# Geronimorz/MCMC-in-Tonga

Measured on AMD Instinct MI355X. Metric: MCMC proposals/sec (likelihood evals/sec) at 381 rays x N cells, higher is better.
Workload: dtype f64

## Files before the change

include/tdstar_testing.h:

```cpp
#ifndef TDSTAR_TESTING_H
#define TDSTAR_TESTING_H
#include <stdint.h>

#include "tdstar.h"

#ifdef __cplusplus
extern "C" {
#endif

void tdt_philox(const uint32_t ctr[4], const uint32_t key[2], uint32_t out[4]);
double tdt_det_log(double x);
double tdt_det_exp(double x);
double tdt_normal_quantile(double p);
void tdt_draws(uint64_t seed, uint32_t chain, uint64_t iter, double out[7]);
int tdt_propose(const td_chain_params *prm, uint64_t iter, int64_t ncells, const double *cx, const double *cy,
                const double *cz, const double *czeta, double czeta_birth, double out[8]);
int tdt_chain_profile(td_chain *ch, int enable, int64_t out[80]);
int tdt_chain_lds(td_chain *ch, int64_t out[4]);
int tdt_chain_variant(const int64_t in[15], int64_t out[8]);
int tdt_chain_variant_rounds(const int64_t in[15], int rounds_rec, int64_t out[8]);
int tdt_chain_launch_counts(int64_t out[32], int *n);
int tdt_chain_draws_launches(int64_t *n);
int tdt_history_pack(int device, double *cells, int64_t stride, int64_t slot0, int64_t slot_cells,
                     const int32_t *ncells, int64_t count, int64_t *off_out);
int tdt_history_pack_chunk(void);
int tdt_chain_query_lat(td_chain *ch, const double *pts, int nq, int mode, int64_t out[4]);
int tdt_tile_filter(const float *lo, const float *hi, const double *maxd, int nt, const double *queries, int nq,
                    int mode, uint8_t *hit);
int tdt_chain_query_answers(td_chain *ch, const double *pts, int nq, int mode, double *dist, double *value,
                            int32_t *proven);
int tdt_accept(const td_chain_params *prm, int action, double u_accept, double zeta_new, int64_t ncells, double phi,
               double phi_n, double czeta, double zeta_killed, double zetanew_death);
int tdt_decide_sure(const td_chain_params *prm, int action, double u_accept, double zeta_new, int64_t ncells,
// ... 64 lines not shown
```

mcmc-in-tonga_amd/_lib.py:

```python
import ctypes
import os

import numpy as np

HERE = os.path.dirname(os.path.abspath(__file__))
LIB_PATH = os.environ.get("TD_LIB_PATH") or os.path.join(HERE, "libtdstar.so")

TD_OK, TD_ERR_ARG, TD_ERR_LAYOUT, TD_ERR_HIP, TD_ERR_NOMEM, TD_ERR_BOUNDS = range(6)
TD_ENGINE_DEVICE, TD_ENGINE_HOST, TD_ENGINE_DROPIN = 0, 1, 2

_d = ctypes.c_double
_i32 = ctypes.c_int32
_i64 = ctypes.c_int64
_u32 = ctypes.c_uint32
_u64 = ctypes.c_uint64
_pd = ctypes.POINTER(ctypes.c_double)
_pi32 = ctypes.POINTER(ctypes.c_int32)
_pi64 = ctypes.POINTER(ctypes.c_int64)
_pu32 = ctypes.POINTER(ctypes.c_uint32)
_vp = ctypes.c_void_p


class TdInfo(ctypes.Structure):
    _fields_ = [("abi_version", _i32), ("device", _i32), ("m", _i64), ("n", _i64), ("npoints", _i64),
# ... 118 lines not shown
    "tdt_set_volume_counting": (ctypes.c_int, [_vp, ctypes.c_int]),
    "tdt_convergence_plan": (ctypes.c_int, [_i64, _pi64, _i64, _pi64, _pi64, _pd]),
    "tdt_set_convergence_round": (ctypes.c_int, [_vp, _i64]),
    "tdt_set_convergence_lag_block": (ctypes.c_int, [_vp, ctypes.c_int]),
    "tdt_quantile_rank": (ctypes.c_int, [_i64, _d, _pi64, _pd]),
    "tdt_set_marginals_method": (ctypes.c_int, [_vp, ctypes.c_int]),
    "tdt_marginals_resident_max": (ctypes.c_int, [_vp, _pi64]),
    "tdt_philox": (None, [_pu32, _pu32, _pu32]),
    "tdt_det_log": (_d, [_d]),
    "tdt_det_exp": (_d, [_d]),
    "tdt_normal_quantile": (_d, [_d]),
    "tdt_draws": (None, [_u64, _u32, _u64, _pd]),
    "tdt_propose": (ctypes.c_int, [ctypes.POINTER(TdChainParams), _u64, _i64, _pd, _pd, _pd, _pd, _d, _pd]),
    "tdt_chain_profile": (ctypes.c_int, [_vp, ctypes.c_int, _pi64]),
    "tdt_chain_lds": (ctypes.c_int, [_vp, _pi64]),
    "tdt_chain_variant": (ctypes.c_int, [_pi64, _pi64]),
    "tdt_chain_variant_rounds": (ctypes.c_int, [_pi64, ctypes.c_int, _pi64]),
    "tdt_chain_launch_counts": (ctypes.c_int, [_pi64, ctypes.POINTER(ctypes.c_int)]),
    "tdt_chain_draws_launches": (ctypes.c_int, [_pi64]),
    "tdt_history_pack": (ctypes.c_int, [ctypes.c_int, _pd, _i64, _i64, _i64, _pi32, _i64, _pi64]),
    "tdt_history_pack_chunk": (ctypes.c_int, []),
    "tdt_chain_query_lat": (ctypes.c_int, [_vp, _pd, ctypes.c_int, ctypes.c_int, _pi64]),
    "tdt_chain_query_answers": (ctypes.c_int, [_vp, _pd, ctypes.c_int, ctypes.c_int, _pd, _pd, _pi32]),
    "tdt_tile_filter": (ctypes.c_int, [ctypes.POINTER(ctypes.c_float), ctypes.POINTER(ctypes.c_float), _pd,
                                       ctypes.c_int, _pd, ctypes.c_int, ctypes.c_int,
                                       ctypes.POINTER(ctypes.c_uint8)]),
    "tdt_set_nn_method": (ctypes.c_int, [_vp, ctypes.c_int]),
    "tdt_nn_bench": (ctypes.c_int, [_vp, _pd, _pd, _pd, _pd, _i64, ctypes.c_int, ctypes.c_int, _pd]),
    "tdt_chain_set_lds_mode": (ctypes.c_int, [_vp, ctypes.c_int]),
    "tdt_chain_set_exact_every": (ctypes.c_int, [_vp, ctypes.c_int]),
# ... 69 lines not shown
```

mcmc-in-tonga_amd/csrc/chain.cpp:

```cpp
#include <hip/hip_runtime.h>

#include <algorithm>
#include <atomic>
#include <chrono>
#include <climits>
#include <cmath>
#include <cstdlib>
#include <cstdio>
#include <cstring>
#include <new>
#include <string>
#include <mutex>
#include <thread>
#include <vector>

#include "../../include/tdstar_testing.h"
#include "chain_dev.h"
#include "chain_logic.h"
#include "comm.h"
#include "ctx.h"
#include "history.h"

using namespace tdstar;

// ... 331 lines not shown
        const int b = grid_bucket(G, ch->x[i], ch->y[i], ch->z[i]);
        if (bcount[(size_t)b] < kBucketCap) {
            bslot[(size_t)b * kBucketCap + bcount[(size_t)b]] = (int)i;
            bent[(size_t)b * kBucketCap + bcount[(size_t)b]++] = CellEntry{ch->x[i], ch->y[i], ch->z[i], ch->zeta[i]};
        }
        else
            overflow = 1;
    }
    size_t bytes = 0;
    auto add = [&](size_t b) { bytes += ((b + 255) / 256) * 256; };
    const size_t Pn = (size_t)std::max<int64_t>(P, 1), nn = (size_t)std::max<int64_t>(n, 1);
    add(sizeof(int) * (ntiles + 1)); add(sizeof(int) * (ntiles + 1)); add(sizeof(int) * Pn);
    add(sizeof(float) * 3 * ntiles); add(sizeof(float) * 3 * ntiles); add(sizeof(double) * (ntiles + 1)); add(sizeof(double) * (ntiles + 1));
    add(sizeof(float) * 3 * std::max(nsuper, 1)); add(sizeof(float) * 3 * std::max(nsuper, 1));
    add(sizeof(double) * 4 * cap); add(sizeof(double) * (cap + 2)); for (int i = 0; i < 3; ++i) add(sizeof(int) * cap); add(sizeof(long long) * cap);
    add(sizeof(int) * Pn); add(sizeof(double) * Pn); add(sizeof(double) * Pn);
    add(sizeof(int) * Pn); add(sizeof(double) * Pn); add(sizeof(double) * Pn); add(Pn);
    add(sizeof(int) * Pn); add(sizeof(int) * Pn); add(sizeof(int) * (ntiles + 1));
    for (int i = 0; i < 6; ++i) add(sizeof(double) * nn);
    add(sizeof(int) * nn); add(sizeof(int) * nn); add(sizeof(ChainScalars));
    add(sizeof(int) * nbuckets); add(sizeof(CellEntry) * nbuckets * kBucketCap); add(sizeof(int) * nbuckets * kBucketCap); add(sizeof(int));
    add(sizeof(DevChain));
    hipError_t e = hipMalloc(&ch->dev_block, bytes);
    if (e != hipSuccess) return hip_err(c, e, "hipMalloc(chain state)");
    e = hipMemsetAsync(ch->dev_block, 0, bytes, c->stream);
    if (e != hipSuccess) return hip_err(c, e, "hipMemset(chain state)");
    char *cur = (char *)ch->dev_block;
    DevChain &d = ch->dev;
    d.px = c->g.px; d.py = c->g.py; d.pz = c->g.pz; d.w = c->g.w; d.tS = c->g.tS; d.sig = c->g.sig;
    d.ray_off = c->g.ray_off;
    d.P = (int)P;
// ... 6 lines not shown
    d.tile_start = tile_start; d.tile_ray = tile_ray_d; d.pt_ray = pt_ray_d; d.tile_lo = tlo; d.tile_hi = thi;
    d.tile_maxd = carve<double>(cur, ntiles + 1);
    d.tile_cmax = carve<double>(cur, ntiles + 1);
    d.ntiles = ntiles;
    float *slo_d = carve<float>(cur, 3 * (size_t)std::max(nsuper, 1));
    float *shi_d = carve<float>(cur, 3 * (size_t)std::max(nsuper, 1));
    d.super_lo = slo_d; d.super_hi = shi_d; d.nsuper = nsuper;
    double *cells = carve<double>(cur, 4 * (size_t)cap);
    d.cx = cells; d.cy = cells + cap; d.cz = cells + 2 * cap; d.czeta = cells + 3 * cap;
    double *logN_d = carve<double>(cur, (size_t)cap + 2);
    d.logN = logN_d;
    d.order = carve<int>(cur, cap); d.stamp = carve<long long>(cur, cap);
    d.free_slots = carve<int>(cur, cap); d.order_tmp = carve<int>(cur, cap);
    d.cap = cap;
    d.best_s = carve<int>(cur, Pn); d.best_d = carve<double>(cur, Pn); d.zeta0 = carve<double>(cur, Pn);
    d.cand_s = carve<int>(cur, Pn); d.cand_d = carve<double>(cur, Pn); d.cand_z = carve<double>(cur, Pn);
    d.cand_flag = carve<unsigned char>(cur, Pn);
    d.changed = carve<int>(cur, Pn); d.orphans = carve<int>(cur, Pn); d.tiles_hit = carve<int>(cur, ntiles + 1);
    d.ptS = carve<double>(cur, nn); d.cand_ptS = carve<double>(cur, nn);
    d.prefix = carve<double>(cur, nn); d.cand_prefix = carve<double>(cur, nn);
    d.term = carve<double>(cur, nn); d.cand_term = carve<double>(cur, nn);
    d.rays_hit = carve<int>(cur, nn); d.ray_flag = carve<int>(cur, nn);
    d.st = carve<ChainScalars>(cur, 1);
    d.grid = G;
    d.bucket_count = carve<int>(cur, nbuckets);
    d.buckets = carve<CellEntry>(cur, nbuckets * kBucketCap);
    d.bslot = carve<int>(cur, nbuckets * kBucketCap);
    d.grid_overflow = carve<int>(cur, 1);
    ch->dev_ptr = carve<DevChain>(cur, 1);
    ch->st_dev = d.st;
// ... 1531 lines not shown
}
int tdt_chain_set_lds_mode(td_chain *ch, int mode) {
    if (!ch || ch->engine != TD_ENGINE_DEVICE || mode < 0 || mode > 3) return TD_ERR_ARG;
    ch->dev.lds_mode = mode;
    ch->desc_dirty = true;
    return TD_OK;
}

int tdt_chain_set_exact_every(td_chain *ch, int k) {
    if (!ch || ch->engine != TD_ENGINE_DEVICE || k < 0) return TD_ERR_ARG;
    ch->dev.exact_every = k;
    ch->desc_dirty = true;
    return TD_OK;
}

int tdt_chain_lds(td_chain *ch, int64_t out[4]) {
    if (!ch || ch->engine != TD_ENGINE_DEVICE || !out) return TD_ERR_ARG;
    chain_lds_sizes(ch->dev, out);
    return TD_OK;
}

int tdt_chain_query_lat(td_chain *ch, const double *pts, int nq, int mode, int64_t out[4]) {
    if (!ch || ch->engine != TD_ENGINE_DEVICE || !pts || nq < 1 || !out) return TD_ERR_ARG;
    td_ctx *c = ch->ctx;
    double *dp = nullptr;
    long long *dout = nullptr;
    hipError_t e = hipMalloc((void **)&dp, sizeof(double) * 3 * (size_t)nq);
    if (e == hipSuccess) e = hipMalloc((void **)&dout, sizeof(long long) * 4);
    if (e == hipSuccess) e = hipMemcpy(dp, pts, sizeof(double) * 3 * (size_t)nq, hipMemcpyHostToDevice);
    if (e == hipSuccess && ch->desc_dirty) {
// ... 117 lines not shown
```

mcmc-in-tonga_amd/csrc/chain_dev.h:

```cpp
#pragma once
#include <hip/hip_runtime.h>

#include <cstddef>
#include <cstdint>

#include "chain_logic.h"
#include "chain_variant.h"
#include "internal.h"
#include "../../include/tdstar.h"

namespace tdstar {

constexpr int kTilePts = 16;
constexpr int kProfSlots = 80;
constexpr int kChainThreads = 512;
constexpr int kBucketCap = 32;
struct CellEntry {
    double x, y, z, zeta;
};

struct ChainScalars {
    int64_t iter;
    int64_t evaluations;
    int64_t accepted[5];
// ... 37 lines not shown
inline void rec_set_slot(RecDesc &r, long long cells) { r.off = reinterpret_cast<long long *>((intptr_t)cells); }

struct DevChain {
    const double *px, *py, *pz, *w, *tS, *sig;
    const int *ray_off, *pt_ray;
    int P, n;
    const int *tile_start;
    const int *tile_ray;
    const float *tile_lo, *tile_hi;
    double *tile_maxd;
    double *tile_cmax;
    int ntiles;
    const float *super_lo, *super_hi;
    int nsuper;
    double *cx, *cy, *cz, *czeta;
    const double *logN;
    int *order, *free_slots, *order_tmp;
    long long *stamp;
    int cap;
    int *best_s;
    double *best_d, *zeta0;
    int *cand_s;
    double *cand_d, *cand_z;
    unsigned char *cand_flag;
    int *changed, *orphans, *tiles_hit;
    double *ptS, *cand_ptS, *prefix, *cand_prefix;
    double *term, *cand_term;
    int *rays_hit;
    int *ray_flag;
    ChainScalars *st;
// ... 147 lines not shown
```

mcmc-in-tonga_amd/csrc/chain_kernels.hip:

```cpp
#pragma clang fp contract(off)

#include <hip/hip_runtime.h>

#include <algorithm>
#include <atomic>
#include <climits>
#include <cstddef>
#include <cstdlib>

#include "chain_dev.h"
#include "chain_diag.h"
#include "chain_resident.h"
#include "chain_search.h"
#include "chain_shared.h"
#include "chain_tiles.h"
#include "chain_variant.h"
#include "exact_sum.h"
#include "internal.h"
#include "ray_sum.h"
#include "wave_ops.h"

namespace tdstar {

namespace {

struct OverlayZeta {
    const unsigned char *flag;
    const double *cand, *cur;
    __device__ __forceinline__ double operator()(int k) const {
        const double a = cand[k], b = cur[k];
        return flag[k] ? a : b;
    }
};

struct ProposalLoads {
    Proposal q;
    int s, new_slot;
    double x, y, z, ze;
};
template <class SlotAt>
__device__ __forceinline__ ProposalLoads proposal_begin(const tdchain::Params &P, const tdchain::Draws &dr,
                                                        int ncells, int nfree, int nslots, const int *free_slots,
                                                        const double *cx, const double *cy, const double *cz,
                                                        const double *czeta, SlotAt slot_at) {
    ProposalLoads l;
    l.q = tdchain::propose(P, dr, ncells);
    l.s = -1;
    l.new_slot = -1;
    l.x = l.y = l.z = l.ze = 0.0;
    if (l.q.active && l.q.action != tdchain::kBirth) {
        l.s = slot_at((int)l.q.index);
        l.x = gload(cx + l.s);
        l.y = gload(cy + l.s);
        l.z = gload(cz + l.s);
        l.ze = gload(czeta + l.s);
    }
    if (l.q.active && l.q.action == tdchain::kBirth) l.new_slot = nfree > 0 ? gload(free_slots + nfree - 1) : nslots;
    return l;
}
__device__ __forceinline__ void proposal_end(PState &o, const tdchain::Params &P, const tdchain::Draws &dr,
                                             ProposalLoads l) {
    Proposal q = l.q;
    o.slot_k = -1;
    o.new_slot = l.new_slot;
    if (q.active && q.action != tdchain::kBirth) {
        o.slot_k = l.s;
        o.kx = l.x;
        o.ky = l.y;
        o.kz = l.z;
        o.zeta_killed = l.ze;
        tdchain::complete_proposal(P, dr, q, l.x, l.y, l.z, l.ze);
    }
    o.p = q;
    o.eval = q.active && (q.valid || q.action == tdchain::kBirth) && P.debug_prior != 1;
}
template <class SlotAt>
__device__ __forceinline__ void make_proposal(PState &o, const tdchain::Params &P, const tdchain::Draws &dr,
                                              int ncells, int nfree, int nslots, const int *free_slots,
                                              const double *cx, const double *cy, const double *cz,
                                              const double *czeta, SlotAt slot_at) {
    proposal_end(o, P, dr, proposal_begin(P, dr, ncells, nfree, nslots, free_slots, cx, cy, cz, czeta, slot_at));
}

template <class SlotAt>
__device__ __forceinline__ void script_proposal(PState &o, const ScriptStep &st, int nfree, int nslots,
                                               const int *free_slots, SlotAt slot_at) {
    Proposal q{};
    q.action = st.action;
    q.active = 1;
    q.valid = 1;
    q.index = st.index;
    q.x = st.x;
    q.y = st.y;
    q.z = st.z;
    q.zeta = st.zeta;
    o.slot_k = -1;
    o.new_slot = -1;
    if (q.action != tdchain::kBirth) {
        const int s = slot_at(st.index);
        o.slot_k = s;
        o.kx = st.old[0];
        o.ky = st.old[1];
        o.kz = st.old[2];
        o.zeta_killed = st.old[3];
        if (q.action == tdchain::kChange) {
            q.x = o.kx;
            q.y = o.ky;
            q.z = o.kz;
        } else if (q.action == tdchain::kMove) {
            q.zeta = o.zeta_killed;
        }
    } else {
// ... 437 lines not shown
        const PState &cur = sh.ps[sh.cur];
        const Proposal p = cur.p;
        const int action = p.action;
        const int ncells = sh.ncells;
        const int slot_k = cur.slot_k;
        const bool eval = cur.eval != 0;
        const double kx = cur.kx, ky = cur.ky, kz = cur.kz;
        const int new_slot = cur.new_slot;
        const double zeta_killed = cur.zeta_killed;
        double czeta = 0.0, zetanew_death = 0.0;
        STAMP(0);
        bool pre_on = false;
        bool nobar = false;
        int pre_q = 0, pre_ray = 0, pre_s = 0;
        double pre_bd = 0.0, pre_x = 0.0, pre_y = 0.0, pre_z = 0.0;
        if (p.active) {
            const bool kill_q = SCRIPT && mb && action == tdchain::kDeath && sh.step_cur.decision == kDecideLater;
            const bool query = (!nscript && (action == tdchain::kBirth || action == tdchain::kDeath)) || kill_q;
            nobar = kNoBarB && action != tdchain::kBirth && p.valid && P.debug_prior != 1;
            if (eval) {
                const bool q0 = action != tdchain::kBirth;
                const bool q1 = action == tdchain::kBirth || action == tdchain::kMove;
                const TileQuery tq0 = tile_query(kx, ky, kz), tq1 = tile_query(p.x, p.y, p.z);
                const int nthr = query ? NTH - 64 : NTH;
                constexpr int TU = SMALL ? 3 : 8;
                if (super_on) {
                    const int par = (int)(it & 1);
                    int *hl = shit + par * kListLds;
                    if (tid < nthr)
                        for (int S0 = tid; S0 < NS; S0 += 4 * nthr) {
                            bool hit[4];
#pragma unroll
                            for (int u = 0; u < 4; ++u) {
                                const int S = min(S0 + u * nthr, NS - 1);
                                const float thr = smax[S] * (1.0f + 0x1p-20f);
// ... 143 lines not shown
            if (RLDS && action == tdchain::kDeath && nscript) {
                const int sthr = query ? NTH - 64 : NTH;
                if constexpr (RLDS) {
                    if (tid < sthr)
                        for (int j = (int)p.index + 1 + tid; j < ncells; j += sthr) d.order_tmp[j] = v.ord[j];
                }
            }
            if (query && wv == kWv - 1) {
                const bool birth = action == tdchain::kBirth;
                if (nobar && lane == 0) atomicAdd(&sh.b_done, 1);
                const Nearest r = wave_nearest(d, v, sh, lane, birth ? p.x : kx, birth ? p.y : ky, birth ? p.z : kz,
                                               birth ? -1 : slot_k, -1, 0.0, 0.0, 0.0, 0.0);
                if (lane == 0) sh.q_zeta = r.z;
            }
        }
        if (!nobar) {
            __syncthreads();
            SKEW(4);
            if (p.active && action == tdchain::kBirth) czeta = sh.q_zeta;
            if (p.active && action == tdchain::kDeath) zetanew_death = sh.q_zeta;
        }
        BPROBE(2);
        Proposal pp = p;
        if (p.active && action == tdchain::kBirth && !nscript) tdchain::birth_zeta(P, pp, czeta);
        STAMP(1);
        const bool can_spec = !nscript && it + 1 < iters && ((it + 1) & 63) != 0;
        if (pp.active && pp.valid) {
            const bool fwd = P.debug_prior != 1;
            int no = 0;
            if (fwd) {
                if (!nscript && tid == NTH - 64)
                    sh.ap = tdchain::alpha_parts(P, pp, czeta, zeta_killed,
                                                 nobar && action == tdchain::kDeath ? sh.q_zeta : zetanew_death,
                                                 sh.lnN);

                const int nt = sh.n_tiles;
                const double zeta_k = slot_k >= 0 ? zeta_killed : 0.0;
                int seen = 0;
                auto point = [&](int q, int ray, int s, double bd, double qx, double qy, double qz) {
                    if (action == tdchain::kBirth) {
                        const double dd = dist2(pp.x, pp.y, pp.z, qx, qy, qz);
                        if (dd < bd) mark(d, v, sh, q, ray, new_slot, dd, pp.zeta);
                    } else if (action == tdchain::kChange) {
                        if (s == slot_k) mark(d, v, sh, q, ray, s, bd, pp.zeta);
                    } else if (s == slot_k) {
                        const int o = atomicAdd(&sh.n_orphans, 1);
                        d.orphans[o] = q;
                        if (o < kOrphanLds) sh.orph[o] = OrphanRec{qx, qy, qz, q, ray};
                    } else if (action == tdchain::kMove) {
                        const double dd = dist2(pp.x, pp.y, pp.z, qx, qy, qz);
                        if (dd < bd || (dd == bd && s >= 0 && d.stamp[slot_k] < d.stamp[s]))
                            mark(d, v, sh, q, ray, slot_k, dd, zeta_k);
                    }
                };
                if constexpr (SMALL) {
                    if (pre_on) {
                        ++seen;
                        point(pre_q, pre_ray, pre_s, pre_bd, pre_x, pre_y, pre_z);
                    }
                    if (nobar)
                        SPIN_WAIT(__hip_atomic_load(&sh.b_done, __ATOMIC_ACQUIRE, __HIP_MEMORY_SCOPE_WORKGROUP) < kWv, 1);
                    const int nt = sh.n_tiles;
                    for (int item = tid; item < nt * kTilePts; item += NTH) {
                        const int t = v.thit[item / kTilePts];
                        if (t < 0) continue;
                        const int sc = v.tstart[t];
                        if (item % kTilePts >= (sc & 31)) continue;
// ... 155 lines not shown
                                            lb = f < lb ? f : lb;
                                        }
                                        if (hi < g - 1) {
                                            const double gap = ((w0 + (double)(hi + 1) * h) - w) - e;
                                            const double f = (gap > 0.0 ? gap * gap : 0.0) + other;
                                            lb = f < lb ? f : lb;
                                        }
                                    };
                                    face(qx, G.x0, G.hx, G.ex, G.gx, i0, i1, o2[1] + o2[2]);
                                    face(qy, G.y0, G.hy, G.ey, G.gy, j0, j1, o2[0] + o2[2]);
                                    face(qz, G.z0, G.hz, G.ez, G.gz, k0b, k1b, o2[0] + o2[1]);
                                    lb = grid_lb_close(lb);
                                    if (bs >= 0 && bd < kSentinel && !tie && bd < lb) {
                                        const int q = o < kOrphanLds ? sh.orph[o].q : d.orphans[o];
                                        const int ray = o < kOrphanLds ? sh.orph[o].ray : d.pt_ray[q];
                                        mark(d, v, sh, q, ray, bs, bd, d.czeta[bs]);
                                    } else {
                                        fb[atomicAdd(&sh.ob_nfb, 1)] = o;
                                    }
                                }
                                __syncthreads();
                                SKEW(9);
                                nlist = sh.ob_nfb;
                                olist = fb;
                            }
                        }
                    }
                }
                for (int k = wv; k < nlist; k += kWv) {
                    const int o = olist ? olist[k] : k;
                    double qx, qy, qz;
// ... 1 lines not shown
                    if (o < kOrphanLds) {
                        qx = sh.orph[o].x;
                        qy = sh.orph[o].y;
                        qz = sh.orph[o].z;
                        q = sh.orph[o].q;
                        ray = sh.orph[o].ray;
                    } else {
                        q = d.orphans[o];
                        qx = d.px[q];
                        qy = d.py[q];
                        qz = d.pz[q];
                        ray = d.pt_ray[q];
                    }
                    const Nearest r =
                        wave_nearest(d, v, sh, lane, qx, qy, qz, skip_s, moved_s, pp.x, pp.y, pp.z, zeta_killed);
                    if (lane == 0) mark(d, v, sh, q, ray, r.s, r.d, r.z);
                }
                if (nlist > 0) __syncthreads();
                SKEW(10);
                STAMP(3);
                const int nr = sh.n_rays;
                const OverlayZeta oz{d.cand_flag, d.cand_z, d.zeta0};
                auto ray_done = [&](int r, double val, double tsr, double sgr, double old_term, int npr) {
                    v.cptS[r] = val;
                    const double df = val - tsr;
                    const double sg = sgr;
                    v.cterm[r] = old_term;
                    const double nterm = ((df * df) * 1.0) / (sg * sg);
                    v.term[r] = nterm;
                    if constexpr (!RLDS) {
                        atomicAdd(&sh.dsum, nterm - old_term);
// ... 223 lines not shown
                    sh.g_op = action == tdchain::kBirth ? 2 : action == tdchain::kDeath ? 1
                              : action == tdchain::kMove ? 3 : 4;
                    sh.g_slot = action == tdchain::kBirth ? new_slot : slot_k;
                    sh.g_ox = kx;
                    sh.g_oy = ky;
                    sh.g_oz = kz;
                    sh.g_nx = pp.x;
                    sh.g_ny = pp.y;
                    sh.g_nz = pp.z;
                    sh.g_nzeta = pp.zeta;
                    if (acc) atomicAdd((unsigned long long *)&sh.accepted[action], 1ull);
                }
                if (prof_on && bdec == 1) atomicAdd((unsigned long long *)&sh.prof[14], 1ull);
            } else if (spec_in_F && tid == 64) {
                if (can_spec) {
                    make_proposal(sh.ps[sh.cur ^ 1], P, draws[(it + 1) & 63], ncells, sh.nfree, sh.nslots, d.free_slots, d.cx,
                                  d.cy, d.cz, d.czeta, [&](int pos) { return v.ord[pos]; });
                    sh.spec_ok = 1;
                }
            } else if (wv == kWv - 1 || (kWv >= 6 && wv == kWv - 2)) {
                if (wv == kWv - 1)
                    grid_prefetch(d, sh, lane, action, action == tdchain::kBirth ? new_slot : slot_k, kx, ky,
                                  kz, pp.x, pp.y, pp.z);
                if (wv == (kWv >= 6 ? kWv - 2 : kWv - 1)) {
                    if (prof_on && lane == 0) {
                        sh.prof[68] += sh.n_tiles;
                        sh.prof[69] += sh.pts_seen;
                        sh.prof[70] += sh.n_changed;
                        sh.prof[71] += sh.n_rays;
                    }
                    if (lane == 0 && fwd) {
                        atomicAdd((unsigned long long *)&sh.evaluations, 1ull);
                        atomicAdd((unsigned long long *)&sh.bytes,
                                  (unsigned long long)((super_on ? (long long)NS * 32 +
                                                                      (long long)sh.n_super[it & 1] * kTilePts * 32
                                                                 : (long long)NT * 32) +
                                                       (long long)sh.pts_seen * 36 +
                                                       (long long)(no + (action <= 2 ? 1 : 0)) * 27 * 8 * 32 +
                                                       (RLDS ? 0ll : (long long)sh.ray_pts * 17) + (long long)(n - sh.k0) * 28));
                    }
                    if (lane == 0 && (action == tdchain::kBirth || action == tdchain::kDeath)) {
                        sh.lnN_far[0] = d.logN[max(ncells - 2, 0)];
                        sh.lnN_far[1] = d.logN[ncells + 2];
                    }
                }
            } else if (wv >= 2 && wv <= (kWv >= 6 ? kWv - 3 : 2) && fwd && action != tdchain::kChange) {
                const int nt = sh.n_tiles;
                constexpr int MU = 4, MS = (kWv >= 6 ? kWv - 4 : 1) * 64;
                if constexpr (RLDS) {
                    for (int i = tid - 128; i < nt * kTilePts; i += MS) {
                        const int sc = v.tile_rec(i / kTilePts).y;
                        const int q = (sc >> 5) + (i % kTilePts);
// ... 40 lines not shown
            __syncthreads();
            STAMP(5);
            SKEW(14);
            const int nc = sh.gs.nc, nr = sh.gs.nr;
            if (nscript && sdec != 1 && !early && wv == 0) server_report(sa.out, v, sh, n, lane, sh.phi_n);
            if (mb && sdec == kDecideLater) {
                if (wv == 0) server_wait(mb, d, v, sh, lane);
                __syncthreads();
                SKEW(15);
                if (tid == 0) acc_r = sh.gs.accept != 0;
            }
            constexpr int kW = NTH - 64;
            const int w = tid - 64;
            if (sh.gs.accept) {
                const int nt = sh.gs.nt, k0 = sh.gs.k0;
                if (wv != 0)
                    for (int c = w; c < nc; c += kW) {
                        if (c < kChgLds) {
                            const ChgRec r = sh.chg[c];
                            d.best_s[r.q] = r.s;
                            d.best_d[r.q] = r.d;
                            d.zeta0[r.q] = r.z;
                            d.cand_flag[r.q] = 0;
                        } else {
                            const int q = d.changed[c];
                            d.best_s[q] = d.cand_s[q];
                            d.best_d[q] = d.cand_d[q];
                            d.zeta0[q] = d.cand_z[q];
                            d.cand_flag[q] = 0;
                        }
                    }
                if (fwd && action != tdchain::kChange) {
                    for (int i = tid; i < nt; i += NTH) v.tmaxd[v.tile_rec(i).x] = v.ctm_at(i);
                    pend_sup = super_on;
                }
                for (int rr = tid; rr < nr; rr += NTH) {
                    const int r = v.ray_at(rr);
                    v.ptS[r] = v.cptS[r];
                    v.rflag[r] = 0;
                }
                if (!WALK || !nscript) {
                    if (!sh.defer)
                        for (int r = k0 + tid; r < n; r += NTH) v.prefix[r] = v.cprefix[r];
                } else if (fwd && k0 < n) {
                    pend_r = true;
                    if (wv == 1) delta_remark(v.term, v.prefix, v.cprefix, n, sh.dseg, smask, lane);
// ... 159 lines not shown
                        if (it + 1 + lane < iters) draws[lane] = sa.pre[(long long)bchain * sa.pre_stride + it + 1 + lane];
                    } else {
                        draws[lane] = tdchain::draw_iteration(d.seed, d.chain, (uint64_t)(iter0 + it + 1 + lane));
                    }
                    wave_sync_lds();
                }
                if (lane == 0) {
                    const bool acc = acc_r;
                    const PState &g = sh.ps[cur_r ^ 1];
                    const bool keep = sh.spec_ok && can_spec &&
                                      (!acc || ((action == tdchain::kChange || action == tdchain::kMove) &&
                                                g.slot_k != slot_k));
                    if (keep) {
                        cur_r ^= 1;
                        sh.cur = cur_r;
                    } else {
                        const bool killed = RLDS && acc && action == tdchain::kDeath;
                        if (killed && !nscript)
                            SPIN_WAIT(__hip_atomic_load(&sh.shift_done, __ATOMIC_ACQUIRE, __HIP_MEMORY_SCOPE_WORKGROUP) <
                                          kWv - 1,
                                      1000000);
                        auto slot_at = [&](int pos) {
                            return (killed && nscript && pos >= (int)pp.index) ? d.order_tmp[pos + 1] : v.ord[pos];
                        };
                        if (nscript) {
                            sh.step_cur = mb ? sh.srv_step[sh.srv_k++] : sa.step[it + 1];
                            script_proposal(sh.ps[cur_r], sh.step_cur, sh.nfree, sh.nslots, d.free_slots, slot_at);
                        }
                        else
                            make_proposal(sh.ps[cur_r], P, draws[(it + 1) & 63], sh.ncells, sh.nfree, sh.nslots,
// ... 252 lines not shown
```

mcmc-in-tonga_amd/csrc/chain_shared.h:

```cpp
#pragma once
#include <hip/hip_runtime.h>

#include <algorithm>
#include <cstddef>

#include "chain_dev.h"
#include "exact_sum.h"
#include "internal.h"

namespace tdstar {

namespace {

using tdchain::Proposal;

constexpr int kWaves = kChainThreads / 64;
static_assert(kTilePts == 16, "a tile is one 16-lane DPP row (row_max_u64)");
constexpr int kOrphanLds = 96;
constexpr int kPre = 64 / kTilePts;
static_assert(kPre == 4, "the preload slots are four registers");
constexpr int kCtmLds = 256;
constexpr int kListLds = 1024;
constexpr int kBatchOrphans = 64;
constexpr int kBatchCand = 192;
constexpr int kBatchBuckets = 512;
constexpr bool kSmallWalk = false;

struct ChgRec {
    int q, s;
    double d, z;
};
constexpr int kChgLds = 64;

struct OrphanRec {
    double x, y, z;
    int q, ray;
};

__device__ __forceinline__ double dist2(double cx, double cy, double cz, double x, double y, double z) {
    const double dx = cx - x, dy = cy - y, dz = cz - z;
    double d = dx * dx;
    d = d + dy * dy;
    d = d + dz * dz;
    return d;
}

template <class R>
__device__ __forceinline__ bool better(double d, R r, double bd, R br) {
    return d < bd || (d == bd && d < kSentinel && r < br);
}

struct PState {
    Proposal p;
    double kx, ky, kz, zeta_killed;
    int slot_k, new_slot, eval;
};

struct GridGeo {
    double x0, y0, z0, ix, iy, iz, hx, hy, hz, ex, ey, ez;
    double lo[3], hi[3];
    double lb0;
    const int *count;
    const CellEntry *buckets;
    const int *bslot;
    int gx, gy, gz, sealed;
};
__device__ __forceinline__ void geo_fill(GridGeo &g, const DevChain &d) {
    const CellGrid &G = d.grid;
    g.x0 = G.x0; g.y0 = G.y0; g.z0 = G.z0;
    g.ix = G.ix; g.iy = G.iy; g.iz = G.iz;
// ... 216 lines not shown
```

mcmc-in-tonga_amd/csrc/chain_state.hip:

```cpp
#pragma clang fp contract(off)

#include <hip/hip_runtime.h>

#include "chain_dev.h"
#include "chain_shared.h"
#include "internal.h"

namespace tdstar {

namespace {

__global__ __launch_bounds__(256) void k_chi2_prefix(const double *__restrict__ ptS, const double *__restrict__ tS,
                                                     const double *__restrict__ sig, int n,
                                                     double *__restrict__ prefix, ChainScalars *st) {
    __shared__ double t[2048];
    double C = 0.0;
    for (int base = 0; base < n; base += 2048) {
        const int cnt = min(2048, n - base);
        for (int k = threadIdx.x; k < cnt; k += 256) {
            const double df = ptS[base + k] - tS[base + k];
            const double sg = sig[base + k];
            t[k] = ((df * df) * 1.0) / (sg * sg);
        }
        __syncthreads();
// ... 5 lines not shown
        __syncthreads();
    }
    if (threadIdx.x == 0) st->phi = C;
}

__global__ void k_tile_max(const int *__restrict__ tile_start, int ntiles, const double *__restrict__ best_d,
                           double *__restrict__ tile_maxd) {
    const int t = blockIdx.x * blockDim.x + threadIdx.x;
    if (t >= ntiles) return;
    double mx = -1.0;
    const int sc = tile_start[t];
    for (int q = sc >> 5; q < (sc >> 5) + (sc & 31); ++q) mx = fmax(mx, best_d[q]);
    tile_maxd[t] = mx;
}

}

hipError_t launch_chi2_prefix(const double *ptS, const double *tS, const double *sig, int n, double *prefix,
                              ChainScalars *st, hipStream_t s) {
    hipLaunchKernelGGL(k_chi2_prefix, dim3(1), dim3(256), 0, s, ptS, tS, sig, n, prefix, st);
    return hipGetLastError();
}

hipError_t chain_full_state(DevChain &d, int ncells, NNWork &work, int num_cus, hipStream_t s) {
    Geometry g;
    g.m = 0;
    g.n = d.n;
    g.P = d.P;
    g.px = const_cast<double *>(d.px);
    g.py = const_cast<double *>(d.py);
    g.pz = const_cast<double *>(d.pz);
    g.w = const_cast<double *>(d.w);
    g.ray_off = const_cast<int *>(d.ray_off);
    g.tS = const_cast<double *>(d.tS);
    g.sig = const_cast<double *>(d.sig);
    hipError_t e = launch_nearest(d.px, d.py, d.pz, d.P, 1, 1, d.cx, d.cap, ncells, work, num_cus, d.best_s,
                                  d.best_d, d.zeta0, s);
    if (e != hipSuccess) return e;
    e = launch_ray_sums(g, d.zeta0, d.ptS, s);
    if (e != hipSuccess) return e;
    e = launch_chi2_prefix(d.ptS, d.tS, d.sig, d.n, d.prefix, d.st, s);
    if (e != hipSuccess) return e;
    if (d.ntiles > 0) {
        hipLaunchKernelGGL(k_tile_max, dim3((d.ntiles + 255) / 256), dim3(256), 0, s, d.tile_start, d.ntiles,
                           d.best_d, d.tile_maxd);
        e = hipGetLastError();
    }
    return e;
}

void chain_lds_sizes(const DevChain &d, int64_t out[4]) {
    const LdsPlan a = lds_plan(d.ntiles, d.n, d.cap, true), b = lds_plan(d.ntiles, d.n, d.cap, false);
    out[0] = (int64_t)a.total;
// ... 7 lines not shown
```

mcmc-in-tonga_amd/csrc/chain_tiles.h:

```cpp
#pragma once
#include <hip/hip_runtime.h>

#include "chain_shared.h"

namespace tdstar {

namespace {

__device__ __forceinline__ void mark(const DevChain &d, const Views &v, Shared &sh, int p, int r, int s, double dd,
                                     double z) {
    d.cand_s[p] = s;
    d.cand_d[p] = dd;
    d.cand_z[p] = z;
    d.cand_flag[p] = 1;
    const int c = atomicAdd(&sh.n_changed, 1);
    d.changed[c] = p;
    if (c < kChgLds) sh.chg[c] = ChgRec{p, s, dd, z};
    if (atomicExch(&v.rflag[r], 1) == 0) {
        v.ray_put(atomicAdd(&sh.n_rays, 1), r);
        atomicMin(&sh.k0, r);
    }
}

struct TileQuery {
    float x, y, z, ex, ey, ez;
};
__device__ __forceinline__ TileQuery tile_query(double x, double y, double z) {
    TileQuery q;
    q.x = (float)x;
    q.y = (float)y;
    q.z = (float)z;
    q.ex = fabsf(q.x) * 0x1p-23f;
// ... 55 lines not shown
```

profiles/chain_phases.py:

```python
#!/usr/bin/env python3
import ctypes
import json
import os
import sys
import time

import numpy as np

ROOT = os.path.dirname(os.path.dirname(os.path.abspath(__file__)))
sys.path.insert(0, ROOT)
import tonga

PHASES = ["(loop top)", "B tiles + birth/death query", "C points", "D orphans", "E ray sums",
          "F chi2 + accept || next proposal, tile maxima", "G commit + grid update + next proposal"]


def main():
    N = int(sys.argv[1]) if len(sys.argv) > 1 else 5000
    iters = int(sys.argv[2]) if len(sys.argv) > 2 else 20000
    nrays = int(sys.argv[3]) if len(sys.argv) > 3 else 0
    tt = tonga.load()
    ds = tt.synthetic_rays(nrays, seed=5) if nrays > 0 else tt.load_data_Tonga()
    ctx = tt.TdContext.from_datastruct(ds)
    prm = tt.define_TDstructrure().replace(max_cells=2 * N)
# ... 26 lines not shown
           "G sub-phases per iter (tid 0)": {
               "commit": round((out[12] - out0[12]) / iters, 1),
               "next proposal": round((out[13] - out0[13]) / iters, 1),
               "final barrier": round((out[6] - out0[6]) / iters, 1)}}
    names = PHASES[:6] + ["G commit", "G next proposal", "final barrier"]
    res["phases_by_action (cycles per proposal)"] = {
        a: {names[j]: round((out[16 + 10 * i + j] - out0[16 + 10 * i + j]) / max(prop[i], 1), 1) for j in range(9)}
        for i, a in enumerate(["birth", "death", "change", "move"])}
    res["F per wave (cycles per iter): chi2 scan, next proposal, tile maxima x4, bound, grid prefetch"] = [
        round((out[56 + w] - out0[56 + w]) / iters, 1) for w in range(8)]
    ev = max(sum(prop), 1)
    res["chi2 tail terms per proposal"] = round((out[64] - out0[64]) / ev, 1)
    res["chi2 scan rounds per proposal"] = round((out[65] - out0[65]) / ev, 2)
    res["per evaluated proposal: tiles hit, points seen, points changed, rays changed"] = [
        round((out[k] - out0[k]) / ev, 1) for k in (68, 69, 70, 71)]
    res["chi2 walk (rays in HBM) per proposal: events, batch-load cycles, walk cycles, terms one by one"] = [
        round((out[k] - out0[k]) / ev, 1) for k in (72, 73, 74, 75)]
    res["F wave 0: cycles to scan end / to decision (per iter)"] = [round((out[k] - out0[k]) / iters, 1)
                                                                     for k in (66, 67)]
    print(json.dumps(res, indent=1))


if __name__ == "__main__":
    main()
```

Baseline: 163,100.

## Track per-cell ray-point ownership counts and skip tile search for barren cells

Keeps a device array counting how many ray points each cell owns as nearest neighbour. It is initialised after the nearest-neighbour build and updated atomically at commit for birth, death and move. The speculative next proposal loads the count, and change or death proposals on a cell that owns no points take a short path. That path skips the tile and point queries, the barrier and the chi2 work, since such a proposal cannot change any ray sum. The cost is extra atomics and a waitcnt at commit, one more load per proposal, and a correctness risk if the counts drift out of sync (a check function is added to test this).

```diff
diff --git a/include/tdstar_testing.h b/include/tdstar_testing.h
--- a/include/tdstar_testing.h
+++ b/include/tdstar_testing.h
@@ -17,6 +17,7 @@
                 const double *cz, const double *czeta, double czeta_birth, double out[8]);
 int tdt_chain_profile(td_chain *ch, int enable, int64_t out[80]);
 int tdt_chain_lds(td_chain *ch, int64_t out[4]);
+int tdt_chain_own_check(td_chain *ch);
 int tdt_chain_variant(const int64_t in[15], int64_t out[8]);
 int tdt_chain_variant_rounds(const int64_t in[15], int rounds_rec, int64_t out[8]);
 int tdt_chain_launch_counts(int64_t out[32], int *n);
diff --git a/mcmc-in-tonga_amd/_lib.py b/mcmc-in-tonga_amd/_lib.py
--- a/mcmc-in-tonga_amd/_lib.py
+++ b/mcmc-in-tonga_amd/_lib.py
@@ -156,6 +156,7 @@
     "tdt_propose": (ctypes.c_int, [ctypes.POINTER(TdChainParams), _u64, _i64, _pd, _pd, _pd, _pd, _d, _pd]),
     "tdt_chain_profile": (ctypes.c_int, [_vp, ctypes.c_int, _pi64]),
     "tdt_chain_lds": (ctypes.c_int, [_vp, _pi64]),
+    "tdt_chain_own_check": (ctypes.c_int, [_vp]),
     "tdt_chain_variant": (ctypes.c_int, [_pi64, _pi64]),
     "tdt_chain_variant_rounds": (ctypes.c_int, [_pi64, ctypes.c_int, _pi64]),
     "tdt_chain_launch_counts": (ctypes.c_int, [_pi64, ctypes.POINTER(ctypes.c_int)]),
diff --git a/mcmc-in-tonga_amd/csrc/chain.cpp b/mcmc-in-tonga_amd/csrc/chain.cpp
--- a/mcmc-in-tonga_amd/csrc/chain.cpp
+++ b/mcmc-in-tonga_amd/csrc/chain.cpp
@@ -369,7 +369,7 @@
     add(sizeof(float) * 3 * ntiles); add(sizeof(float) * 3 * ntiles); add(sizeof(double) * (ntiles + 1)); add(sizeof(double) * (ntiles + 1));
     add(sizeof(float) * 3 * std::max(nsuper, 1)); add(sizeof(float) * 3 * std::max(nsuper, 1));
     add(sizeof(double) * 4 * cap); add(sizeof(double) * (cap + 2)); for (int i = 0; i < 3; ++i) add(sizeof(int) * cap); add(sizeof(long long) * cap);
-    add(sizeof(int) * Pn); add(sizeof(double) * Pn); add(sizeof(double) * Pn);
+    add(sizeof(int) * Pn); add(sizeof(double) * Pn); add(sizeof(double) * Pn); add(sizeof(int) * cap);
     add(sizeof(int) * Pn); add(sizeof(double) * Pn); add(sizeof(double) * Pn); add(Pn);
     add(sizeof(int) * Pn); add(sizeof(int) * Pn); add(sizeof(int) * (ntiles + 1));
     for (int i = 0; i < 6; ++i) add(sizeof(double) * nn);
@@ -406,6 +406,7 @@
     d.free_slots = carve<int>(cur, cap); d.order_tmp = carve<int>(cur, cap);
     d.cap = cap;
     d.best_s = carve<int>(cur, Pn); d.best_d = carve<double>(cur, Pn); d.zeta0 = carve<double>(cur, Pn);
+    d.own = carve<int>(cur, cap);
     d.cand_s = carve<int>(cur, Pn); d.cand_d = carve<double>(cur, Pn); d.cand_z = carve<double>(cur, Pn);
     d.cand_flag = carve<unsigned char>(cur, Pn);
     d.changed = carve<int>(cur, Pn); d.orphans = carve<int>(cur, Pn); d.tiles_hit = carve<int>(cur, ntiles + 1);
@@ -1967,6 +1968,28 @@
     return TD_OK;
 }
 
+int tdt_chain_own_check(td_chain *ch) {
+    if (!ch || ch->engine != TD_ENGINE_DEVICE) return -TD_ERR_ARG;
+    if (ch->prm.debug_prior == 1) return 0;
+    td_ctx *c = ch->ctx;
+    const DevChain &d = ch->dev;
+    std::vector<int> bs((size_t)std::max(d.P, 0)), own((size_t)d.cap), cnt((size_t)d.cap, 0);
+    hipError_t e = hipStreamSynchronize(c->stream);
+    if (e == hipSuccess && !bs.empty()) e = hipMemcpy(bs.data(), d.best_s, sizeof(int) * bs.size(), hipMemcpyDeviceToHost);
+    if (e == hipSuccess && !own.empty()) e = hipMemcpy(own.data(), d.own, sizeof(int) * own.size(), hipMemcpyDeviceToHost);
+    if (e != hipSuccess) {
+        hip_err(c, e, "tdt_chain_own_check");
+        return -TD_ERR_HIP;
+    }
+    int bad = 0;
+    for (int s : bs) {
+        if (s >= 0 && s < d.cap) cnt[(size_t)s] += 1;
+        else bad += 1;
+    }
+    for (int s = 0; s < d.cap; ++s) bad += own[(size_t)s] != cnt[(size_t)s];
+    return bad;
+}
+
 int tdt_chain_lds(td_chain *ch, int64_t out[4]) {
     if (!ch || ch->engine != TD_ENGINE_DEVICE || !out) return TD_ERR_ARG;
     chain_lds_sizes(ch->dev, out);
diff --git a/mcmc-in-tonga_amd/csrc/chain_dev.h b/mcmc-in-tonga_amd/csrc/chain_dev.h
--- a/mcmc-in-tonga_amd/csrc/chain_dev.h
+++ b/mcmc-in-tonga_amd/csrc/chain_dev.h
@@ -75,6 +75,7 @@
     const float *super_lo, *super_hi;
     int nsuper;
     double *cx, *cy, *cz, *czeta;
+    int *own;
     const double *logN;
     int *order, *free_slots, *order_tmp;
     long long *stamp;
diff --git a/mcmc-in-tonga_amd/csrc/chain_kernels.hip b/mcmc-in-tonga_amd/csrc/chain_kernels.hip
--- a/mcmc-in-tonga_amd/csrc/chain_kernels.hip
+++ b/mcmc-in-tonga_amd/csrc/chain_kernels.hip
@@ -36,17 +36,20 @@
 struct ProposalLoads {
     Proposal q;
     int s, new_slot;
+    int own;
     double x, y, z, ze;
 };
-template <class SlotAt>
+template <bool OWN = false, class SlotAt>
 __device__ __forceinline__ ProposalLoads proposal_begin(const tdchain::Params &P, const tdchain::Draws &dr,
                                                         int ncells, int nfree, int nslots, const int *free_slots,
                                                         const double *cx, const double *cy, const double *cz,
-                                                        const double *czeta, SlotAt slot_at) {
+                                                        const double *czeta, SlotAt slot_at,
+                                                        const int *own = nullptr) {
     ProposalLoads l;
     l.q = tdchain::propose(P, dr, ncells);
     l.s = -1;
     l.new_slot = -1;
+    l.own = -1;
     l.x = l.y = l.z = l.ze = 0.0;
     if (l.q.active && l.q.action != tdchain::kBirth) {
         l.s = slot_at((int)l.q.index);
@@ -54,6 +57,9 @@
         l.y = gload(cy + l.s);
         l.z = gload(cz + l.s);
         l.ze = gload(czeta + l.s);
+        if constexpr (OWN)
+            l.own = __hip_atomic_load((const __attribute__((address_space(1))) int *)(own + l.s), __ATOMIC_RELAXED,
+                                      __HIP_MEMORY_SCOPE_AGENT);
     }
     if (l.q.active && l.q.action == tdchain::kBirth) l.new_slot = nfree > 0 ? gload(free_slots + nfree - 1) : nslots;
     return l;
@@ -63,6 +69,7 @@
     Proposal q = l.q;
     o.slot_k = -1;
     o.new_slot = l.new_slot;
+    o.barren = l.own == 0 ? 1 : 0;
     if (q.active && q.action != tdchain::kBirth) {
         o.slot_k = l.s;
         o.kx = l.x;
@@ -74,12 +81,12 @@
     o.p = q;
     o.eval = q.active && (q.valid || q.action == tdchain::kBirth) && P.debug_prior != 1;
 }
-template <class SlotAt>
+template <bool OWN = false, class SlotAt>
 __device__ __forceinline__ void make_proposal(PState &o, const tdchain::Params &P, const tdchain::Draws &dr,
                                               int ncells, int nfree, int nslots, const int *free_slots,
                                               const double *cx, const double *cy, const double *cz,
-                                              const double *czeta, SlotAt slot_at) {
-    proposal_end(o, P, dr, proposal_begin(P, dr, ncells, nfree, nslots, free_slots, cx, cy, cz, czeta, slot_at));
+                                              const double *czeta, SlotAt slot_at, const int *own = nullptr) {
+    proposal_end(o, P, dr, proposal_begin<OWN>(P, dr, ncells, nfree, nslots, free_slots, cx, cy, cz, czeta, slot_at, own));
 }
 
 template <class SlotAt>
@@ -96,6 +103,7 @@
     q.zeta = st.zeta;
     o.slot_k = -1;
     o.new_slot = -1;
+    o.barren = 0;
     if (q.action != tdchain::kBirth) {
         const int s = slot_at(st.index);
         o.slot_k = s;
@@ -563,11 +571,13 @@
         bool nobar = false;
         int pre_q = 0, pre_ray = 0, pre_s = 0;
         double pre_bd = 0.0, pre_x = 0.0, pre_y = 0.0, pre_z = 0.0;
+        const bool sroad = !SCRIPT && cur.barren != 0 && p.active && p.valid && P.debug_prior != 1 &&
+                           (action == tdchain::kChange || action == tdchain::kDeath);
         if (p.active) {
             const bool kill_q = SCRIPT && mb && action == tdchain::kDeath && sh.step_cur.decision == kDecideLater;
             const bool query = (!nscript && (action == tdchain::kBirth || action == tdchain::kDeath)) || kill_q;
-            nobar = kNoBarB && action != tdchain::kBirth && p.valid && P.debug_prior != 1;
-            if (eval) {
+            nobar = kNoBarB && action != tdchain::kBirth && p.valid && P.debug_prior != 1 && !sroad;
+            if (eval && !sroad) {
                 const bool q0 = action != tdchain::kBirth;
                 const bool q1 = action == tdchain::kBirth || action == tdchain::kMove;
                 const TileQuery tq0 = tile_query(kx, ky, kz), tq1 = tile_query(p.x, p.y, p.z);
@@ -741,7 +751,7 @@
                 if (lane == 0) sh.q_zeta = r.z;
             }
         }
-        if (!nobar) {
+        if (!nobar && !(sroad && action == tdchain::kChange)) {
             __syncthreads();
             SKEW(4);
             if (p.active && action == tdchain::kBirth) czeta = sh.q_zeta;
@@ -755,7 +765,7 @@
         if (pp.active && pp.valid) {
             const bool fwd = P.debug_prior != 1;
             int no = 0;
-            if (fwd) {
+            if (fwd && !sroad) {
                 if (!nscript && tid == NTH - 64)
                     sh.ap = tdchain::alpha_parts(P, pp, czeta, zeta_killed,
                                                  nobar && action == tdchain::kDeath ? sh.q_zeta : zetanew_death,
@@ -767,9 +777,9 @@
                 auto point = [&](int q, int ray, int s, double bd, double qx, double qy, double qz) {
                     if (action == tdchain::kBirth) {
                         const double dd = dist2(pp.x, pp.y, pp.z, qx, qy, qz);
-                        if (dd < bd) mark(d, v, sh, q, ray, new_slot, dd, pp.zeta);
+                        if (dd < bd) mark(d, v, sh, q, ray, new_slot, dd, pp.zeta, s);
                     } else if (action == tdchain::kChange) {
-                        if (s == slot_k) mark(d, v, sh, q, ray, s, bd, pp.zeta);
+                        if (s == slot_k) mark(d, v, sh, q, ray, s, bd, pp.zeta, s);
                     } else if (s == slot_k) {
                         const int o = atomicAdd(&sh.n_orphans, 1);
                         d.orphans[o] = q;
@@ -777,7 +787,7 @@
                     } else if (action == tdchain::kMove) {
                         const double dd = dist2(pp.x, pp.y, pp.z, qx, qy, qz);
                         if (dd < bd || (dd == bd && s >= 0 && d.stamp[slot_k] < d.stamp[s]))
-                            mark(d, v, sh, q, ray, slot_k, dd, zeta_k);
+                            mark(d, v, sh, q, ray, slot_k, dd, zeta_k, s);
                     }
                 };
                 if constexpr (SMALL) {
@@ -963,7 +973,7 @@
                                     if (bs >= 0 && bd < kSentinel && !tie && bd < lb) {
                                         const int q = o < kOrphanLds ? sh.orph[o].q : d.orphans[o];
                                         const int ray = o < kOrphanLds ? sh.orph[o].ray : d.pt_ray[q];
-                                        mark(d, v, sh, q, ray, bs, bd, d.czeta[bs]);
+                                        mark(d, v, sh, q, ray, bs, bd, d.czeta[bs], slot_k);
                                     } else {
                                         fb[atomicAdd(&sh.ob_nfb, 1)] = o;
                                     }
@@ -995,7 +1005,7 @@
                     }
                     const Nearest r =
                         wave_nearest(d, v, sh, lane, qx, qy, qz, skip_s, moved_s, pp.x, pp.y, pp.z, zeta_killed);
-                    if (lane == 0) mark(d, v, sh, q, ray, r.s, r.d, r.z);
+                    if (lane == 0) mark(d, v, sh, q, ray, r.s, r.d, r.z, slot_k);
                 }
                 if (nlist > 0) __syncthreads();
                 SKEW(10);
@@ -1249,8 +1259,8 @@
                 if (prof_on && bdec == 1) atomicAdd((unsigned long long *)&sh.prof[14], 1ull);
             } else if (spec_in_F && tid == 64) {
                 if (can_spec) {
-                    make_proposal(sh.ps[sh.cur ^ 1], P, draws[(it + 1) & 63], ncells, sh.nfree, sh.nslots, d.free_slots, d.cx,
-                                  d.cy, d.cz, d.czeta, [&](int pos) { return v.ord[pos]; });
+                    make_proposal<true>(sh.ps[sh.cur ^ 1], P, draws[(it + 1) & 63], ncells, sh.nfree, sh.nslots,
+                                        d.free_slots, d.cx, d.cy, d.cz, d.czeta, [&](int pos) { return v.ord[pos]; }, d.own);
                     sh.spec_ok = 1;
                 }
             } else if (wv == kWv - 1 || (kWv >= 6 && wv == kWv - 2)) {
@@ -1259,6 +1269,7 @@
                                   kz, pp.x, pp.y, pp.z);
                 if (wv == (kWv >= 6 ? kWv - 2 : kWv - 1)) {
                     if (prof_on && lane == 0) {
+                        if (sroad) sh.prof[action == tdchain::kDeath ? 35 : 45] += 1;
                         sh.prof[68] += sh.n_tiles;
                         sh.prof[69] += sh.pts_seen;
                         sh.prof[70] += sh.n_changed;
@@ -1266,11 +1277,14 @@
                     }
                     if (lane == 0 && fwd) {
                         atomicAdd((unsigned long long *)&sh.evaluations, 1ull);
+                        const bool owns_none = !SCRIPT && ((action == tdchain::kChange && sh.n_changed == 0) ||
+                                                          (action == tdchain::kDeath && no == 0));
                         atomicAdd((unsigned long long *)&sh.bytes,
-                                  (unsigned long long)((super_on ? (long long)NS * 32 +
-                                                                      (long long)sh.n_super[it & 1] * kTilePts * 32
-                                                                 : (long long)NT * 32) +
-                                                       (long long)sh.pts_seen * 36 +
+                                  (unsigned long long)((owns_none  ? 0ll
+                                                        : super_on ? (long long)NS * 32 +
+                                                                         (long long)sh.n_super[it & 1] * kTilePts * 32 +
+                                                                         (long long)sh.pts_seen * 36
+                                                                   : (long long)NT * 32 + (long long)sh.pts_seen * 36) +
                                                        (long long)(no + (action <= 2 ? 1 : 0)) * 27 * 8 * 32 +
                                                        (RLDS ? 0ll : (long long)sh.ray_pts * 17) + (long long)(n - sh.k0) * 28));
                     }
@@ -1341,22 +1355,34 @@
             const int w = tid - 64;
             if (sh.gs.accept) {
                 const int nt = sh.gs.nt, k0 = sh.gs.k0;
-                if (wv != 0)
+                if (wv != 0) {
+                    const bool owners = action != tdchain::kChange;
                     for (int c = w; c < nc; c += kW) {
+                        int so, sn;
                         if (c < kChgLds) {
                             const ChgRec r = sh.chg[c];
                             d.best_s[r.q] = r.s;
                             d.best_d[r.q] = r.d;
                             d.zeta0[r.q] = r.z;
                             d.cand_flag[r.q] = 0;
+                            so = r.o;
+                            sn = r.s;
                         } else {
                             const int q = d.changed[c];
-                            d.best_s[q] = d.cand_s[q];
+                            so = d.best_s[q];
+                            sn = d.cand_s[q];
+                            d.best_s[q] = sn;
                             d.best_d[q] = d.cand_d[q];
                             d.zeta0[q] = d.cand_z[q];
                             d.cand_flag[q] = 0;
                         }
-                    }
+                        if (owners && so != sn) {
+                            if (so >= 0) atomicAdd(&d.own[so], -1);
+                            if (sn >= 0) atomicAdd(&d.own[sn], 1);
+                        }
+                    }
+                    if (owners && w < nc) __builtin_amdgcn_s_waitcnt(0);
+                }
                 if (fwd && action != tdchain::kChange) {
                     for (int i = tid; i < nt; i += NTH) v.tmaxd[v.tile_rec(i).x] = v.ctm_at(i);
                     pend_sup = super_on;
@@ -1546,6 +1572,11 @@
                     if (keep) {
                         cur_r ^= 1;
                         sh.cur = cur_r;
+                        if (prof_on && g.barren) sh.prof[55] += 1;
+                        if (acc && action != tdchain::kChange && sh.gs.nc != 0) {
+                            if (prof_on && g.barren) sh.prof[25] += 1;
+                            sh.ps[cur_r].barren = 0;
+                        }
                     } else {
                         const bool killed = RLDS && acc && action == tdchain::kDeath;
                         if (killed && !nscript)
diff --git a/mcmc-in-tonga_amd/csrc/chain_shared.h b/mcmc-in-tonga_amd/csrc/chain_shared.h
--- a/mcmc-in-tonga_amd/csrc/chain_shared.h
+++ b/mcmc-in-tonga_amd/csrc/chain_shared.h
@@ -29,6 +29,7 @@
 struct ChgRec {
     int q, s;
     double d, z;
+    int o;
 };
 constexpr int kChgLds = 64;
 
@@ -54,6 +55,7 @@
     Proposal p;
     double kx, ky, kz, zeta_killed;
     int slot_k, new_slot, eval;
+    int barren;
 };
 
 struct GridGeo {
diff --git a/mcmc-in-tonga_amd/csrc/chain_state.hip b/mcmc-in-tonga_amd/csrc/chain_state.hip
--- a/mcmc-in-tonga_amd/csrc/chain_state.hip
+++ b/mcmc-in-tonga_amd/csrc/chain_state.hip
@@ -43,6 +43,13 @@
     tile_maxd[t] = mx;
 }
 
+__global__ __launch_bounds__(256) void k_own_count(const int *__restrict__ best_s, int P, int cap, int *__restrict__ own) {
+    const int q = blockIdx.x * blockDim.x + threadIdx.x;
+    if (q >= P) return;
+    const int s = best_s[q];
+    if (s >= 0 && s < cap) atomicAdd(&own[s], 1);
+}
+
 }
 
 hipError_t launch_chi2_prefix(const double *ptS, const double *tS, const double *sig, int n, double *prefix,
@@ -66,6 +73,13 @@
     hipError_t e = launch_nearest(d.px, d.py, d.pz, d.P, 1, 1, d.cx, d.cap, ncells, work, num_cus, d.best_s,
                                   d.best_d, d.zeta0, s);
     if (e != hipSuccess) return e;
+    e = hipMemsetAsync(d.own, 0, sizeof(int) * (size_t)d.cap, s);
+    if (e != hipSuccess) return e;
+    if (d.P > 0) {
+        hipLaunchKernelGGL(k_own_count, dim3((d.P + 255) / 256), dim3(256), 0, s, d.best_s, d.P, d.cap, d.own);
+        e = hipGetLastError();
+        if (e != hipSuccess) return e;
+    }
     e = launch_ray_sums(g, d.zeta0, d.ptS, s);
     if (e != hipSuccess) return e;
     e = launch_chi2_prefix(d.ptS, d.tS, d.sig, d.n, d.prefix, d.st, s);
diff --git a/mcmc-in-tonga_amd/csrc/chain_tiles.h b/mcmc-in-tonga_amd/csrc/chain_tiles.h
--- a/mcmc-in-tonga_amd/csrc/chain_tiles.h
+++ b/mcmc-in-tonga_amd/csrc/chain_tiles.h
@@ -8,14 +8,14 @@
 namespace {
 
 __device__ __forceinline__ void mark(const DevChain &d, const Views &v, Shared &sh, int p, int r, int s, double dd,
-                                     double z) {
+                                     double z, int o) {
     d.cand_s[p] = s;
     d.cand_d[p] = dd;
     d.cand_z[p] = z;
     d.cand_flag[p] = 1;
     const int c = atomicAdd(&sh.n_changed, 1);
     d.changed[c] = p;
-    if (c < kChgLds) sh.chg[c] = ChgRec{p, s, dd, z};
+    if (c < kChgLds) sh.chg[c] = ChgRec{p, s, dd, z, o};
     if (atomicExch(&v.rflag[r], 1) == 0) {
         v.ray_put(atomicAdd(&sh.n_rays, 1), r);
         atomicMin(&sh.k0, r);
diff --git a/profiles/chain_phases.py b/profiles/chain_phases.py
--- a/profiles/chain_phases.py
+++ b/profiles/chain_phases.py
@@ -64,6 +64,11 @@
     res["chi2 scan rounds per proposal"] = round((out[65] - out0[65]) / ev, 2)
     res["per evaluated proposal: tiles hit, points seen, points changed, rays changed"] = [
         round((out[k] - out0[k]) / ev, 1) for k in (68, 69, 70, 71)]
+    short = [int(out[k] - out0[k]) for k in (35, 45)]
+    res["short road (the cell owns no ray point): deaths, changes, share of all proposals"] = short + [
+        round(sum(short) / ev, 4)]
+    res["guesses adopted with a barren cell, of those with the flag cleared at adoption"] = [
+        int(out[k] - out0[k]) for k in (55, 25)]
     res["chi2 walk (rays in HBM) per proposal: events, batch-load cycles, walk cycles, terms one by one"] = [
         round((out[k] - out0[k]) / ev, 1) for k in (72, 73, 74, 75)]
     res["F wave 0: cycles to scan end / to decision (per iter)"] = [round((out[k] - out0[k]) / iters, 1)
```

Result: faster. 166,600, median of 6 (+2.2%).
